# YJxyzxyz/road-vision-system

Hardware: AMD Instinct MI355X
Metric: end-to-end frames/sec @1080p (preproc+YOLOv8n+SORT), 1/2/4/8 MI355X (higher is better)
Workload: dtype bf16

## Files before the change

road-vision-system_amd/csrc/conv.h:

```cpp
#pragma once
#include "common.h"

namespace rv {

typedef uint16_t bf16_t;

struct ConvArgs {
  const bf16_t* in;
  int in_cs, in_co;
  int Hin, Win, Cin;
  const bf16_t* w;
  const float* bias;
  int Cout, k, stride, pad;
  int Ho, Wo, B;
  void* out0;
  int out0_cs, out0_co, out0_up;
  void* out1;
  int out1_cs, out1_co, out1_up;
  int out_f32;
  const bf16_t* res;
  int res_cs, res_co;
  int act;
  int g2_cout0, g2_in_co, g2_Cin;
  const bf16_t* g2_w;
  const float* g2_bias;
  int fused;
  int in8, out0_8, out1_8;
  float s_in, s_res, s_out0, s_out1;
  const float* wscale;
  const float* g2_wscale;
  const bf16_t* in2;
  int in2_cs, in2_co, split, in_up;
  const bf16_t* ch_w;
  const float* ch_b;
};

struct ConvCfg {
  int mr, nr, G, resw, persist;
  int kind = 0;
};

int launch_conv(const ConvArgs& a, hipStream_t s);
int launch_conv_cfg(const ConvArgs& a, const ConvCfg& c, hipStream_t s);
bool conv_cfg_ok(const ConvArgs& a, const ConvCfg& c);
int conv_candidates(const ConvArgs& a, ConvCfg* out, int cap);

struct Conv0Q {
  const int8_t* d;
  const float* s;
  const float* b;
  const int32_t* c;
};
int launch_conv0(const uint8_t* img, int B, int H, int W, const Conv0Q& q, int C0, bf16_t* out,
                 int out_cs, hipStream_t s);
int launch_conv0_fp8(const uint8_t* img, int B, int H, int W, const Conv0Q& q, int C0,
                     uint8_t* out, int out_cs, float s_out, hipStream_t s);

int launch_conv0_k6(const uint8_t* img, int B, int H, int W, const Conv0Q& q, int C0, bf16_t* out,
                    int out_cs, hipStream_t s);

int launch_stem(const uint8_t* img, int B, int H, int W, const Conv0Q& q0, int C0,
                const bf16_t* w1, const float* b1, int C1, bf16_t* out, int out_cs,
                hipStream_t s, const bf16_t* w2 = nullptr, const float* b2 = nullptr,
                bf16_t* out2 = nullptr, int out2_cs = 0, bool k6 = false);

int launch_sppf_pool(bf16_t* buf, int B, int H, int W, int c, hipStream_t s);
int launch_sppf_pool_fp8(uint8_t* buf, int B, int H, int W, int c, hipStream_t s);

struct C2fArgs {
  const bf16_t* cat;
  int cat_cs, cat_co;
  int H, W, B;
  const bf16_t* wa[2];
  const float* ba[2];
  const bf16_t* wb[2];
  const float* bb[2];
  const bf16_t* w2;
  const float* b2;
  bf16_t* out;
  int out_cs, out_co;
  int tap_pairs;
};
bool c2f_fusable(int C, int N, int cat_cs, int cat_co, int out_cs, int out_co);
int launch_c2f_chain(const C2fArgs& a, int C, int N, bool shortcut, hipStream_t s);

struct HeadLevel {
  const float* logits;
  int H, W, cs;
  float stride;
  const bf16_t* feat;
  int feat_cs, cin_b, cin_c;
  const bf16_t* w_box;
  const bf16_t* w_cls;
  const float* b_box;
  const float* b_cls;
  float* logits_out;
};

struct Cand {
  float x1, y1, x2, y2, score;
  int cls, anchor, pad;
};

int decode_segments(const HeadLevel* lv, int nlv);
int launch_detect_decode(const HeadLevel* lv, int nlv, int B, int nc, int reg_max, float conf,
                         float* raw, Cand* cand, int cand_cap, int* seg_n, hipStream_t s,
                         int* form = nullptr, bool cls_only = false);

struct HeadBoxLevel {
  const bf16_t* t;
  int t_cs;
  const bf16_t* w1;
  const float* b1;
};
int launch_head_box(const HeadLevel* lv, const HeadBoxLevel* bx, int nlv, int B, int reg_max,
                    Cand* cand, int cand_cap, const int* seg_n, hipStream_t s);

}
```

road-vision-system_amd/csrc/head_box.hip:

```cpp
#include "conv.h"
#include "conv_common.h"
#include "head.h"

namespace rv {

struct HeadBoxLevels {
  HeadBoxLevel lv[4];
};

constexpr int kBoxC = 64;
constexpr int kURow = kBoxC + 8;
constexpr int kWRowB = 9 * kBoxC * 2 + 16;
constexpr int kWUnits = 9 * kBoxC * 2 / 16;
constexpr int kWPerThread = kBoxC * kWUnits / 256;

template <int REG>
__global__ __launch_bounds__(256) void head_box_kernel(HeadLevels h, HeadBoxLevels hb, int B,
                                                       Cand* __restrict__ cand, int cap,
                                                       const int* __restrict__ seg_n, int nblk) {
  static_assert(4 * REG == kBoxC, "box branch width");
  static_assert(kBoxC * kWUnits % 256 == 0, "weight staging: whole units per thread");
  constexpr int MB = kBoxC / 16, KB = kBoxC / 32;
  extern __shared__ __attribute__((aligned(16))) uint8_t wlds[];
  __shared__ int soff[65];
// ... 28 lines not shown
    b1v[m] = *(const f32x4*)(X.b1 + m * 16 + quad * 4);
    b2v[m] = *(const f32x4*)(L.b_box + m * 16 + quad * 4);
  }
  int n0 = wave == 0 && lane < nsegl ? seg_n[(size_t)b * nblk + blk0 + lane] : 0;
  {
    uint4 wr[kWPerThread];
#pragma unroll
    for (int j = 0; j < kWPerThread; ++j)
      wr[j] = *(const uint4*)(X.w1 + (size_t)(tid + j * 256) * 8);
#pragma unroll
    for (int j = 0; j < kWPerThread; ++j) {
      const int u = tid + j * 256;
      *(uint4*)(wlds + (u / kWUnits) * kWRowB + (u % kWUnits) * 16) = wr[j];
    }
  }
  for (int c0 = 0; c0 < nsegl; c0 += 64) {
    if (wave == 0) {
      const int sgi = c0 + lane;
      int n = c0 == 0 ? n0 : (sgi < nsegl ? seg_n[(size_t)b * nblk + blk0 + sgi] : 0);
      n = min(max(n, 0), 64);
      n = min(n, max(cap - (blk0 + sgi) * 64, 0));
#pragma unroll
      for (int off = 1; off < 64; off <<= 1) {
        const int o = __shfl_up(n, off);
        if (lane >= off) n += o;
      }
      soff[lane + 1] = n;
      if (lane == 0) soff[0] = 0;
    }
    __syncthreads();
    for (int e = tid; e < 64 * 64; e += 256) {
      const int o = soff[e >> 6];
      if ((e & 63) < soff[(e >> 6) + 1] - o) list[o + (e & 63)] = (uint16_t)e;
    }
    __syncthreads();
    const int total = soff[64];
    Cand* const cbase = cand + (size_t)b * cap + (size_t)(blk0 + c0) * 64;
    for (int g0 = z * 4; g0 * 16 < total; g0 += 4 * nz) {
      const int g = g0 + wave;
      const bool active = g * 16 < total;
      int x = 0, y = 0, slot = 0;
      uint4 Bf[KB * 9];
      if (active) {
        const int ci = g * 16 + col;
        slot = list[ci < total ? ci : g * 16];
        int r = cbase[slot].anchor - lstart;
        r = min(max(r, 0), HW - 1);
        y = r / W;
        x = r - y * W;
#pragma unroll
        for (int t = 0; t < 9; ++t) {
          const int yy = y + t / 3 - 1, xx = x + t % 3 - 1;
          const bool in = yy >= 0 && yy < H && xx >= 0 && xx < W;
          const bf16_t* p = tmap + (size_t)(in ? yy * W + xx : 0) * X.t_cs + quad * 8;
#pragma unroll
          for (int k = 0; k < KB; ++k)
            Bf[k * 9 + t] = in ? *(const uint4*)(p + k * 32) : make_uint4(0, 0, 0, 0);
        }
      }
      if (active) {
        f32x4 acc[MB];
#pragma unroll
        for (int m = 0; m < MB; ++m) acc[m] = f32x4{0.f, 0.f, 0.f, 0.f};
#pragma unroll
        for (int k = 0; k < KB; ++k)
#pragma unroll
          for (int t = 0; t < 9; ++t)
#pragma unroll
            for (int m = 0; m < MB; ++m) {
              const uint4 Af = *(const uint4*)(wlds + (m * 16 + col) * kWRowB +
                                               ((t * kBoxC + k * 32 + quad * 8) * 2));
              acc[m] = __builtin_amdgcn_mfma_f32_16x16x32_bf16(
                  __builtin_bit_cast(bf16x8, Af), __builtin_bit_cast(bf16x8, Bf[k * 9 + t]), acc[m],
                  0, 0, 0);
            }
#pragma unroll
        for (int m = 0; m < MB; ++m) {
          float v[4];
#pragma unroll
          for (int i = 0; i < 4; ++i) v[i] = acc[m][i] + b1v[m][i];
          silu4(v);
          *(uint2*)(uw + col * kURow + m * 16 + quad * 4) =
              make_uint2(pack_bf16x2(v[0], v[1]), pack_bf16x2(v[2], v[3]));
        }
      }
      __syncthreads();
      if (active) {
        f32x4 acc[MB];
#pragma unroll
        for (int m = 0; m < MB; ++m) acc[m] = f32x4{0.f, 0.f, 0.f, 0.f};
#pragma unroll
        for (int k = 0; k < KB; ++k) {
          const uint4 Bu = *(const uint4*)(uw + col * kURow + k * 32 + quad * 8);
#pragma unroll
          for (int m = 0; m < MB; ++m)
            acc[m] = __builtin_amdgcn_mfma_f32_16x16x32_bf16(__builtin_bit_cast(bf16x8, Aw[k][m]),
                                                             __builtin_bit_cast(bf16x8, Bu), acc[m],
                                                             0, 0, 0);
        }
#pragma unroll
        for (int m = 0; m < MB; ++m)
          *(f32x4*)(lw + col * (kBoxC + 4) + m * 16 + quad * 4) = acc[m] + b2v[m];
      }
      __syncthreads();
      if (active) {
        const int an = lane >> 2, part = lane & 3;
        const float d = dfl_side<REG>(lw + an * (kBoxC + 4) + part * REG);
        const int base = lane & ~3;
        const float d0 = __shfl(d, base), d1 = __shfl(d, base + 1), d2 = __shfl(d, base + 2),
                    d3 = __shfl(d, base + 3);
        const int xa = __shfl(x, an), ya = __shfl(y, an), sa = __shfl(slot, an);
        if (part == 0 && g * 16 + an < total)
          *(f32x4*)&cbase[sa].x1 = xywh2xyxy(dist2bbox(d0, d1, d2, d3, xa, ya, L.stride));
      }
    }
    __syncthreads();
  }
}

int launch_head_box(const HeadLevel* lv, const HeadBoxLevel* bx, int nlv, int B, int reg_max,
                    Cand* cand, int cand_cap, const int* seg_n, hipStream_t s) {
  HeadLevels h;
  if (!head_levels(lv, nlv, reg_max, h)) return RV_EINVAL;
  HeadBoxLevels hb = {};
  for (int i = 0; i < nlv; ++i) {
    if (!lv[i].w_box || !lv[i].b_box || lv[i].cin_b != kBoxC || !bx[i].t || !bx[i].w1 ||
        !bx[i].b1 || bx[i].t_cs % 8 || (uintptr_t)bx[i].t % 16 || (uintptr_t)bx[i].w1 % 16 ||
        (uintptr_t)bx[i].b1 % 16) {
      set_error("sparse box branch: bad level %d (box width %d)", i, lv[i].cin_b);
      return RV_EINVAL;
    }
    hb.lv[i] = bx[i];
  }
  const int nblk = h.blk[nlv];
  if (!cand || !seg_n || B < 1 || cand_cap < 1 || (uintptr_t)cand % 16) {
    set_error("sparse box branch: candidate buffers incomplete");
    return RV_EINVAL;
  }
  constexpr int smem = kBoxC * kWRowB;
  static const bool raised =
      hipFuncSetAttribute((const void*)head_box_kernel<16>,
                          hipFuncAttributeMaxDynamicSharedMemorySize, smem) == hipSuccess;
  if (!raised) {
    (void)hipGetLastError();
    set_error("sparse box branch: cannot raise the dynamic LDS limit to %d bytes", smem);
    return RV_EINVAL;
  }
  int nz = 4;
  while (nz > 1 && (long)nlv * B * nz > 2L * num_cus()) nz >>= 1;
  head_box_kernel<16><<<dim3(nlv, B, nz), 256, smem, s>>>(h, hb, B, cand, cand_cap, seg_n, nblk);
  return launch_status("head_box");
}

}
```

road-vision-system_amd/csrc/yolo.hip:

```cpp
#include <cmath>
#include <cstring>
#include "yolo_model.h"

namespace rv {

static void plan_heads(Model& M) {
  const Variant& v = M.def.v;
  for (int i = 0; i < 3; ++i) {
    const std::string l = std::to_string(i);
    M.DA[i] = M.newbuf("DA" + l, 3 + i, v.c2d + v.c3p);
    M.DB[i] = M.newbuf("DB" + l, 3 + i, v.c2d + v.c3p, false, true);
    M.HD[i] = M.newbuf("HD" + l, 3 + i, v.hcs, true);
  }
  M.nA = M.map_h[3] * M.map_w[3] + M.map_h[4] * M.map_w[4] + M.map_h[5] * M.map_w[5];
}

static void plan_v5u(Model& M) {
  const Variant& v = M.def.v;
  M.CAT14 = M.CAT11 = -1;
  M.X0 = M.newbuf("X0", 1, v.c1);
  M.X1 = M.newbuf("X1", 2, v.c2);
  M.C2 = M.newbuf("C2", 2, v.c2);
  M.X2 = M.newbuf("X2", 2, v.c2);
  M.X3 = M.newbuf("X3", 3, v.c3);
  M.C4 = M.newbuf("C4", 3, v.c3);
  M.X4 = M.newbuf("X4", 3, v.c3);
  M.X5 = M.newbuf("X5", 4, v.c4);
  M.C6 = M.newbuf("C6", 4, v.c4);
  M.X6 = M.newbuf("X6", 4, v.c4);
  M.X7 = M.newbuf("X7", 5, v.c5);
  M.C8 = M.newbuf("C8", 5, v.c5);
  M.X8 = M.newbuf("X8", 5, v.c5);
  M.SP = M.newbuf("SP", 5, 4 * (v.c5 / 2));
  M.X9 = M.newbuf("X9", 5, v.c5);
  M.CAT20 = M.newbuf("CAT20", 5, 2 * v.c4);
  M.C12 = M.newbuf("C12", 4, v.c4);
  M.X13 = M.newbuf("X13", 4, v.c4);
  M.CAT17 = M.newbuf("CAT17", 4, 2 * v.c3);
  M.C15 = M.newbuf("C15", 3, v.c3);
  M.X15 = M.newbuf("X15", 3, v.c3);
  M.C18 = M.newbuf("C18", 4, v.c4);
  M.X18 = M.newbuf("X18", 4, v.c4);
  M.C21 = M.newbuf("C21", 5, v.c5);
  M.X21 = M.newbuf("X21", 5, v.c5);
  plan_heads(M);
  struct C3Def {
    const char* p;
    int level, c2, n;
  };
  const C3Def cs[] = {{"model.2", 2, v.c2, v.nb},  {"model.4", 3, v.c3, v.nm},
                      {"model.6", 4, v.c4, v.nx},  {"model.8", 5, v.c5, v.nb},
                      {"model.13", 4, v.c4, v.nb}, {"model.17", 3, v.c3, v.nb},
                      {"model.20", 4, v.c4, v.nb}, {"model.23", 5, v.c5, v.nb}};
  for (const C3Def& c : cs)
    for (int i = 0; i < c.n; ++i) {
      M.newbuf(std::string(c.p) + ".t." + std::to_string(i), c.level, c.c2 / 2);
      M.newbuf(std::string(c.p) + ".m." + std::to_string(i), c.level, c.c2 / 2);
    }
}

static void plan(Model& M) {
  const Variant& v = M.def.v;
  for (int i = 0; i < 6; ++i) {
    M.map_h[i] = M.H >> i;
    M.map_w[i] = M.W >> i;
  }
  if (v.family == kFamilyV5u) return plan_v5u(M);
  M.X0 = M.newbuf("X0", 1, v.c1);
  M.X1 = M.newbuf("X1", 2, v.c2);
  M.C2 = M.newbuf("C2", 2, (2 + v.nb) * (v.c2 / 2));
  M.X2 = M.newbuf("X2", 2, v.c2);
  M.X3 = M.newbuf("X3", 3, v.c3);
  M.C4 = M.newbuf("C4", 3, (2 + v.nm) * (v.c3 / 2));
  M.CAT14 = M.newbuf("CAT14", 3, v.h12 + v.c3);
  M.X5 = M.newbuf("X5", 4, v.c4);
  M.C6 = M.newbuf("C6", 4, (2 + v.nm) * (v.c4 / 2));
  M.CAT11 = M.newbuf("CAT11", 4, v.c5 + v.c4);
  M.X7 = M.newbuf("X7", 5, v.c5);
  M.C8 = M.newbuf("C8", 5, (2 + v.nb) * (v.c5 / 2));
  M.X8 = M.newbuf("X8", 5, v.c5);
  M.SP = M.newbuf("SP", 5, 4 * (v.c5 / 2));
  M.CAT20 = M.newbuf("CAT20", 5, v.h18 + v.c5);
  M.C12 = M.newbuf("C12", 4, (2 + v.nb) * (v.h12 / 2));
  M.CAT17 = M.newbuf("CAT17", 4, v.h15 + v.h12);
  M.C15 = M.newbuf("C15", 3, (2 + v.nb) * (v.h15 / 2));
  M.X15 = M.newbuf("X15", 3, v.h15);
  M.C18 = M.newbuf("C18", 4, (2 + v.nb) * (v.h18 / 2));
  M.X18 = M.newbuf("X18", 4, v.h18);
  M.C21 = M.newbuf("C21", 5, (2 + v.nb) * (v.h21 / 2));
  M.X21 = M.newbuf("X21", 5, v.h21);
  plan_heads(M);
  struct C2fDef {
    const char* p;
    int level, c2, n;
  };
  const C2fDef cs[] = {{"model.2", 2, v.c2, v.nb},  {"model.4", 3, v.c3, v.nm},
                       {"model.6", 4, v.c4, v.nm},  {"model.8", 5, v.c5, v.nb},
                       {"model.12", 4, v.h12, v.nb}, {"model.15", 3, v.h15, v.nb},
                       {"model.18", 4, v.h18, v.nb}, {"model.21", 5, v.h21, v.nb}};
  for (const C2fDef& c : cs)
    for (int i = 0; i < c.n; ++i)
      M.newbuf(std::string(c.p) + ".m." + std::to_string(i), c.level, c.c2 / 2);
}

static const View NO_VIEW{-1, 0, 0};

constexpr float kSparseAutoConf = 0.1f;
constexpr int kSparseAutoBatch = 8;

struct ConvIO {
  View in;
  int li;
  View o0;
  int up0 = 0;
  View o1 = NO_VIEW;
  int up1 = 0;
  View res = NO_VIEW;
  const VIn* vin = nullptr;
};

struct Exec {
  Model* M;
  uint8_t* ws;
  int B;
  hipStream_t s;
  std::vector<size_t> off;
  int status = 0;
  bool f8, fusing;
  bool fuse_c2f, fuse_c2f32;
  int cat14, cat11, cat20, cat17;

  Exec(Model* m, void* ws_, int B_, void* stream, std::vector<size_t> off_, bool raw)
      : M(m), ws((uint8_t*)ws_), B(B_), s(as_stream(stream)), off(std::move(off_)) {
    const Variant& v = M->def.v;
    f8 = M->def.dtype == RV_YOLO_DTYPE_FP8;
    fusing = !f8 && !(raw && M->raw_unfused);
    fuse_c2f = fusing && M->fuse_c2f;
    fuse_c2f32 = fuse_c2f && M->fuse_c2f == 2;
    cat14 = v.h12 + v.c3, cat11 = v.c5 + v.c4, cat20 = v.h18 + v.c5, cat17 = v.h15 + v.h12;
    if (v.family == kFamilyV5u) cat14 = cat17 = 2 * v.c3, cat11 = cat20 = 2 * v.c4;
  }

  void* ptr(int buf) const { return ws + off[buf]; }
  const bf16_t* wptr(const ConvSpec& c) const { return (const bf16_t*)(M->dev + c.w_off); }
  const float* bptr(const ConvSpec& c) const { return (const float*)(M->dev + c.b_off); }
  const float* wsptr(const ConvSpec& c) const {
    return c.f8 ? (const float*)(M->dev + c.ws_off) : nullptr;
  }
  float scale(int buf) const { return buf >= 0 ? M->act_scale[buf] : 1.0f; }

  const ConvSpec* spec(const std::string& name) {
    const int idx = M->def.find(name);
    if (idx < 0 && !status) {
      set_error("plan: unknown conv %s", name.c_str());
      status = RV_EINVAL;
    }
    return idx < 0 ? nullptr : &M->def.convs[idx];
  }
  int index(const ConvSpec& c) const { return (int)(&c - M->def.convs.data()); }

  static int out_dim(const ConvSpec& c, int n) { return (n + 2 * (c.k / 2) - c.k) / c.s + 1; }

  ConvArgs args(const ConvSpec& c, const ConvIO& io) const {
    const View in = io.vin ? io.vin->a : io.in, o0 = io.o0, o1 = io.o1, res = io.res;
    ConvArgs a = {};
    a.in = (const bf16_t*)ptr(in.buf);
    a.in_cs = in.cs;
    a.in_co = in.co;
    a.Hin = M->map_h[io.li];
    a.Win = M->map_w[io.li];
    a.Cin = c.pcin;
    a.w = wptr(c);
    a.bias = bptr(c);
    a.Cout = c.pcout;
    a.k = c.k;
    a.stride = c.s;
    a.pad = c.k / 2;
    a.Ho = out_dim(c, a.Hin);
    a.Wo = out_dim(c, a.Win);
    a.B = B;
    a.out0 = ptr(o0.buf);
    a.out0_cs = o0.cs;
    a.out0_co = o0.co;
    a.out0_up = io.up0;
    if (o1.buf >= 0) {
      a.out1 = ptr(o1.buf);
      a.out1_cs = o1.cs;
      a.out1_co = o1.co;
      a.out1_up = io.up1;
    }
    a.out_f32 = M->bufs[o0.buf].f32 ? 1 : 0;
    if (res.buf >= 0) {
      a.res = (const bf16_t*)ptr(res.buf);
      a.res_cs = res.cs;
      a.res_co = res.co;
    }
    a.act = c.act;
    if (c.f8) {
      a.in8 = 1;
      a.s_in = scale(in.buf);
      a.wscale = wsptr(c);
      a.out0_8 = M->bufs[o0.buf].esize == 1;
      a.s_out0 = scale(o0.buf);
      if (o1.buf >= 0) {
        a.out1_8 = M->bufs[o1.buf].esize == 1;
        a.s_out1 = scale(o1.buf);
      }
      if (res.buf >= 0) a.s_res = scale(res.buf);
    }
    if (io.vin) {
      a.in_up = io.vin->up;
      a.in2 = (const bf16_t*)ptr(io.vin->b.buf);
      a.in2_cs = io.vin->b.cs;
      a.in2_co = io.vin->b.co;
      a.split = io.vin->split;
    }
    return a;
  }

  void trace(const ConvSpec& c, const ConvIO& io) {
    const VIn* vi = io.vin;
    const int Hin = M->map_h[io.li], Win = M->map_w[io.li];
    M->trace.push_back(TraceRec{index(c), vi ? vi->a : io.in, Hin, Win, out_dim(c, Hin),
                                out_dim(c, Win), io.o0, io.up0, io.o1, io.up1, io.res,
                                vi ? vi->up : 0, vi ? vi->b : NO_VIEW, vi ? vi->split : 0});
  }

  static double launch_bytes(const ConvArgs& a) {
    const double px_in = (double)a.B * a.Hin * a.Win, px_out = (double)a.B * a.Ho * a.Wo;
    if (a.split > 0 || a.in_up) {
      const double cin1 = a.split > 0 ? a.split : a.Cin;
      const double src = (a.in_up ? px_in / 4 : px_in) * cin1 + px_in * (a.Cin - cin1);
      const double outs = (a.out0 ? (a.out0_up ? 4 : 1) : 0) + (a.out1 ? (a.out1_up ? 4 : 1) : 0);
      return 2.0 * src + 2.0 * px_out * a.Cout * outs + 2.0 * a.Cout * a.Cin;
    }
    const bool g2 = a.g2_cout0 > 0;
    const int cout1 = g2 ? a.g2_cout0 : a.Cout, cout2 = g2 ? a.Cout - a.g2_cout0 : 0;
    double in_ch = a.Cin;
    if (g2 && (a.g2_in_co != a.in_co || a.g2_Cin != a.Cin)) in_ch += a.g2_Cin;
    const double eb = a.in8 ? 1.0 : 2.0;
    auto ob = [&](int o8) { return a.out_f32 ? 4.0 : (o8 ? 1.0 : 2.0); };
    const double outs = (a.out0 ? (a.out0_up ? 4 : 1) * ob(a.out0_8) : 0) +
                        (a.out1 ? (a.out1_up ? 4 : 1) * ob(a.out1_8) : 0);
    const double w = eb * a.k * a.k * ((double)cout1 * a.Cin + (double)cout2 * (g2 ? a.g2_Cin : 0)) +
                     (a.ch_w ? 2.0 * a.Cout * a.Cout : 0.0);
    return px_in * in_ch * eb + px_out * a.Cout * outs + (a.res ? px_out * a.Cout * eb : 0.0) + w;
  }

  double flops_of(const ConvSpec& c, int li) const {
    return 2.0 * B * out_dim(c, M->map_h[li]) * out_dim(c, M->map_w[li]) * (double)c.cout * c.cin *
           c.k * c.k;
  }

  void launch(const ConvArgs& a, const ConvSpec& c, double flops, double bytes) {
    const int li_ = M->li_base + (int)M->launches.size();
    M->launches.push_back(a);
    status = M->prof.timed(li_, s, index(c), flops, bytes, [&] {
      if (a.fused > 0) {
        const Model::FusedC2f& f = M->fused[a.fused - 1];
        return launch_c2f_chain(f.a, f.C, f.N, f.shortcut, s);
      }
// ... 158 lines not shown
  Model* M = E.M;
  const Variant& v = M->def.v;
  const View x0{M->X0, v.c1, 0}, x1{M->X1, v.c2, 0}, x2{M->X2, v.c2, 0};
  const ConvSpec& c0 = M->def.convs[0];
  const uint8_t* qb = M->dev + M->def.q_off;
  const float* qs = (const float*)(qb + 9 * (size_t)c0.cout * 64);
  const Conv0Q q0{(const int8_t*)qb, qs, qs + c0.cout, (const int32_t*)(qs + 2 * c0.cout)};
  const double px0 = (double)E.B * M->map_h[1] * M->map_w[1];
  const double px1 = (double)E.B * M->map_h[2] * M->map_w[2];
  const double f0 = 2.0 * px0 * c0.cout * 108, by_in = (double)E.B * M->H * M->W * 3 + M->def.q_bytes;
  const int slot = M->prof.per_fwd - 1;
  const int i1 = M->def.find("model.1");
  if (E.fusing && M->stem6_fused && c0.cout == 16 && v.c2 == 32 && i1 >= 0) {
    const ConvSpec& c1 = M->def.convs[i1];
    E.trace(c1, {x0, 1, x1});
    E.status = M->prof.timed(slot, E.s, 0, f0 + 2.0 * px1 * c1.cout * c1.cin * 9,
                             by_in + px1 * 2.0 * c1.cout + 2.0 * c1.cout * 9 * 32, [&] {
                               return launch_stem(lb, E.B, M->H, M->W, q0, c0.cout, E.wptr(c1),
                                                  E.bptr(c1), c1.cout, (bf16_t*)E.ptr(M->X1), v.c2,
                                                  E.s, nullptr, nullptr, nullptr, 0, true);
                             });
  } else {
    E.status = M->prof.timed(slot, E.s, 0, f0, by_in + px0 * 2.0 * c0.cout, [&] {
      return launch_conv0_k6(lb, E.B, M->H, M->W, q0, c0.cout, (bf16_t*)E.ptr(M->X0), v.c1, E.s);
    });
    E.conv("model.1", {x0, 1, x1});
  }
  E.c3("model.2", {x1, 2, x2}, M->C2, v.c2, v.nb, true);
  return E.status;
}

static int seg_backbone_v5u(Exec& E) {
  Model* M = E.M;
  const Variant& v = M->def.v;
  const int sc = v.c5 / 2;
  const View x2{M->X2, v.c2, 0}, x3{M->X3, v.c3, 0}, p3{M->X4, v.c3, 0}, x5{M->X5, v.c4, 0},
      p4{M->X6, v.c4, 0}, x7{M->X7, v.c5, 0}, x8{M->X8, v.c5, 0}, sp{M->SP, 4 * sc, 0},
      x9{M->X9, v.c5, 0}, x13{M->X13, v.c4, 0};
  const View t10{M->CAT20, E.cat20, v.c4}, t14{M->CAT17, E.cat17, v.c3};
  const VIn vin13{t10, 1, p4, v.c4}, vin17{t14, 1, p3, v.c3};
  E.conv("model.3", {x2, 2, x3});
  E.c3("model.4", {x3, 3, p3}, M->C4, v.c3, v.nm, true);
  E.conv("model.5", {p3, 3, x5});
  E.c3("model.6", {x5, 4, p4}, M->C6, v.c4, v.nx, true);
  E.conv("model.7", {p4, 4, x7});
  E.c3("model.8", {x7, 5, x8}, M->C8, v.c5, v.nb, true);
  E.conv("model.9.cv1", {x8, 5, sp});
  if (!E.status)
    E.status = launch_sppf_pool((bf16_t*)E.ptr(M->SP), E.B, M->map_h[5], M->map_w[5], sc, E.s);
  E.conv("model.9.cv2", {sp, 5, x9});
  E.conv("model.10", {x9, 5, t10});
  E.c3("model.13", {t10, 4, x13, 0, NO_VIEW, 0, NO_VIEW, &vin13}, M->C12, v.c4, v.nb, false);
  E.conv("model.14", {x13, 4, t14});
  E.c3("model.17", {t14, 3, View{M->X15, v.h15, 0}, 0, NO_VIEW, 0, NO_VIEW, &vin17}, M->C15, v.c3,
       v.nb, false);
  return E.status;
}

static int seg_stem(Exec& E, const uint8_t* lb) {
  Model* M = E.M;
  const Variant& v = M->def.v;
  const int B = E.B;
  const View x0{M->X0, v.c1, 0}, x1{M->X1, v.c2, 0}, x2{M->X2, v.c2, 0};
  const ConvSpec& c0 = M->def.convs[0];
  const uint8_t* qb = M->dev + M->def.q_off;
  const float* qs = (const float*)(qb + 3 * (size_t)c0.cout * 64);
  const Conv0Q q0{(const int8_t*)qb, qs, qs + c0.cout, (const int32_t*)(qs + 2 * c0.cout)};
  const int i1 = M->def.find("model.1");
  const bool fuse_stem = E.fusing && c0.cout == 16 && v.c2 == 32 && i1 >= 0;
  const int i2cv1 = M->def.find("model.2.cv1");
  const int c2cs = E.c2f_will_fuse(v.c2 / 2, v.nb, E.fuse_c2f, 0, NO_VIEW, x2)
                       ? v.c2
                       : (2 + v.nb) * (v.c2 / 2);
  const bool stem_cv1 = fuse_stem && i2cv1 >= 0 && M->def.convs[i2cv1].cin == 32 &&
                        M->def.convs[i2cv1].cout == 32 && M->def.convs[i2cv1].k == 1;
  if (fuse_stem) {
    const ConvSpec& c1 = M->def.convs[i1];
    E.trace(c1, {x0, 1, x1});
    const ConvSpec* cv = stem_cv1 ? &M->def.convs[i2cv1] : nullptr;
    if (cv) E.trace(*cv, {x1, 2, View{M->C2, c2cs, 0}});
    const bool x1_out = !cv || M->stem_x1;
    const double px0 = (double)B * M->map_h[1] * M->map_w[1];
    const double px1 = (double)B * M->map_h[2] * M->map_w[2];
    const double flops = 2.0 * px0 * c0.cout * 27 + 2.0 * px1 * c1.cout * c1.cin * 9 +
                         (cv ? 2.0 * px1 * cv->cout * cv->cin : 0.0);
    const double bytes = (double)B * M->H * M->W * 3 + px1 * 2.0 * (x1_out ? c1.cout : 0) +
                         (cv ? px1 * 2.0 * cv->cout : 0.0) + M->def.q_bytes +
                         2.0 * c1.cout * 9 * 32 + (cv ? 2.0 * cv->cout * 32 : 0.0);
    E.status = M->prof.timed(M->prof.per_fwd - 1, E.s, 0, flops, bytes, [&] {
      return launch_stem(lb, B, M->H, M->W, q0, c0.cout, E.wptr(c1), E.bptr(c1), c1.cout,
                         x1_out ? (bf16_t*)E.ptr(M->X1) : nullptr, v.c2, E.s,
                         cv ? E.wptr(*cv) : nullptr, cv ? E.bptr(*cv) : nullptr,
                         cv ? (bf16_t*)E.ptr(M->C2) : nullptr, c2cs);
    });
  } else {
    E.status = E.f8 ? launch_conv0_fp8(lb, B, M->H, M->W, q0, c0.cout, (uint8_t*)E.ptr(M->X0),
                                       v.c1, E.scale(M->X0), E.s)
                    : launch_conv0(lb, B, M->H, M->W, q0, c0.cout, (bf16_t*)E.ptr(M->X0), v.c1,
                                   E.s);
    E.conv("model.1", {x0, 1, x1});
  }
  E.c2f("model.2", {x1, 2, x2}, M->C2, v.c2, v.nb, true, E.fuse_c2f, stem_cv1);
  return E.status;
}

static int seg_backbone(Exec& E) {
  Model* M = E.M;
  const Variant& v = M->def.v;
  const int cat14 = E.cat14, cat11 = E.cat11, sc = v.c5 / 2;
  const View x2{M->X2, v.c2, 0}, x3{M->X3, v.c3, 0}, x5{M->X5, v.c4, 0}, x7{M->X7, v.c5, 0},
      x8{M->X8, v.c5, 0}, sp{M->SP, 4 * sc, 0};
  const View p3{M->CAT14, cat14, v.h12}, p4{M->CAT11, cat11, v.c5}, p5{M->CAT20, E.cat20, v.h18},
      n4{M->CAT17, E.cat17, v.h15}, c11{M->CAT11, cat11, 0}, c14{M->CAT14, cat14, 0};
  const bool vcat = !E.f8;
  const VIn vin12{p5, 1, p4, v.c5}, vin15{n4, 1, p3, v.h12};
  const int c4 = v.c3 / 2;
  const bool f4 = c4 == 16 ? E.fuse_c2f : E.fuse_c2f32;
  const int c4cs = E.c2f_will_fuse(c4, v.nm, f4, 0, NO_VIEW, p3) ? 2 * c4 : (2 + v.nm) * c4;
  const bool chained = M->fuse_cv1 && E.fusing &&
                       E.conv_chain("model.3", x2, 2, x3, "model.4.cv1", View{M->C4, c4cs, 0});
  if (!chained) E.conv("model.3", {x2, 2, x3});
  E.c2f("model.4", {x3, 3, p3}, M->C4, v.c3, v.nm, true, f4, chained);
  E.conv("model.5", {p3, 3, x5});
  E.c2f("model.6", {x5, 4, p4}, M->C6, v.c4, v.nm, true);
  E.conv("model.7", {p4, 4, x7});
  E.c2f("model.8", {x7, 5, x8}, M->C8, v.c5, v.nb, true);
  E.conv("model.9.cv1", {x8, 5, sp});
  if (!E.status)
    E.status =
        E.f8 ? launch_sppf_pool_fp8((uint8_t*)E.ptr(M->SP), E.B, M->map_h[5], M->map_w[5], sc, E.s)
             : launch_sppf_pool((bf16_t*)E.ptr(M->SP), E.B, M->map_h[5], M->map_w[5], sc, E.s);
  E.conv("model.9.cv2", {sp, 5, p5, 0, vcat ? NO_VIEW : c11, vcat ? 0 : 1});
  E.c2f("model.12", {c11, 4, n4, 0, vcat ? NO_VIEW : c14, vcat ? 0 : 1, NO_VIEW, vcat ? &vin12 : nullptr},
        M->C12, v.h12, v.nb, false);
  E.c2f("model.15", {c14, 3, View{M->X15, v.h15, 0}, 0, NO_VIEW, 0, NO_VIEW, vcat ? &vin15 : nullptr},
        M->C15, v.h15, v.nb, false, v.h15 / 2 == 16 ? E.fuse_c2f : E.fuse_c2f32);
  return E.status;
}

static int seg_heads(Exec& E, float* raw_out, float conf, void* cand, int cand_cap, int* cand_n) {
  Model* M = E.M;
  const Variant& v = M->def.v;
  const int B = E.B;
  const View c17{M->CAT17, E.cat17, 0}, c20{M->CAT20, E.cat20, 0};
  const View P[3] = {View{M->X15, v.h15, 0}, View{M->X18, v.h18, 0}, View{M->X21, v.h21, 0}};
  const int dcs = v.c2d + v.c3p, hcs = v.hcs;
  const bool fuse_head = v.c2d % 8 == 0 && v.c3p % 8 == 0;
  const bool fork =
      M->head_streams && B >= 8 && M->side[0] && M->side[1] && !M->prof.active();
  const hipStream_t main_s = E.s;
  const bool fixed_head = fuse_head && !E.f8 && !raw_out && cand && v.c2d == 64 &&
                          (v.nc == 80 || v.nc <= 64) && v.c3p == (v.nc == 80 ? 80 : 64);
  const bool sparse =
      fixed_head && (M->head_sparse == 1 ||
                     (M->head_sparse == 2 && conf >= kSparseAutoConf && B >= kSparseAutoBatch));
  HeadLevel hl[3] = {};
  HeadBoxLevel hbx[3] = {};
  auto head_level = [&](int i) {
    const std::string a = M->def.head + "cv2." + std::to_string(i),
                      c = M->def.head + "cv3." + std::to_string(i);
    const View da{M->DA[i], dcs, 0}, fb{M->DB[i], dcs, 0}, fc{M->DB[i], dcs, v.c2d},
        lg{M->HD[i], hcs, 0};
    E.conv_pair(a + ".0", P[i], c + ".0", P[i], 3 + i, da);
    if (sparse) {
      const ConvSpec* p1 = E.spec(a + ".1");
      if (!p1) return E.status;
      E.conv_in_sparse(a + ".1", {da, 3 + i, fb});
      E.conv(c + ".1", {View{M->DA[i], dcs, v.c2d}, 3 + i, fc});
      hbx[i] = HeadBoxLevel{(const bf16_t*)E.ptr(M->DA[i]), dcs, E.wptr(*p1), E.bptr(*p1)};
    } else {
      E.conv_pair(a + ".1", da, c + ".1", View{M->DA[i], dcs, v.c2d}, 3 + i, fb);
    }
    HeadLevel& L = hl[i];
    L.logits = (const float*)E.ptr(M->HD[i]);
    L.H = M->map_h[3 + i];
    L.W = M->map_w[3 + i];
    L.cs = hcs;
    L.stride = (float)(8 << i);
    if (!fuse_head) {
      E.conv_pair(a + ".2", fb, c + ".2", fc, 3 + i, lg);
      return E.status;
    }
    const ConvSpec *pa = E.spec(a + ".2"), *pc = E.spec(c + ".2");
    if (!pa || !pc) return E.status;
    const ConvSpec &sa = *pa, &sc = *pc;
    E.trace(sa, {fb, 3 + i, lg});
    E.trace(sc, {fc, 3 + i, View{M->HD[i], hcs, 4 * v.reg}});
    L.feat = (const bf16_t*)E.ptr(M->DB[i]);
    L.feat_cs = dcs;
    L.cin_b = sa.pcin;
    L.cin_c = sc.pcin;
    L.w_box = E.wptr(sa);
    L.w_cls = E.wptr(sc);
    L.b_box = E.bptr(sa);
    L.b_cls = E.bptr(sc);
    L.logits_out = raw_out ? (float*)E.ptr(M->HD[i]) : nullptr;
    return E.status;
  };
  auto forked_head = [&](int i) {
    if (!fork) return head_level(i);
    int e = hip_check(hipEventRecord(M->ev_fork[i], main_s), "head fork hipEventRecord");
    if (!e) e = hip_check(hipStreamWaitEvent(M->side[i], M->ev_fork[i], 0), "head fork wait");
    if (e) return E.status = e;
    E.s = M->side[i];
    const int r = head_level(i);
    e = hip_check(hipEventRecord(M->ev_join[i], M->side[i]), "head join hipEventRecord");
    E.s = main_s;
    if (!r && e) E.status = e;
    return r ? r : e;
  };
  const bool v5 = v.family == kFamilyV5u;
  if (E.status || forked_head(0)) return E.status;
  E.conv(v5 ? "model.18" : "model.16", {P[0], 3, c17});
  if (v5)
    E.c3("model.20", {c17, 4, P[1]}, M->C18, v.h18, v.nb, false);
  else
    E.c2f("model.18", {c17, 4, P[1]}, M->C18, v.h18, v.nb, false);
  if (E.status || forked_head(1)) return E.status;
  E.conv(v5 ? "model.21" : "model.19", {P[1], 4, c20});
  if (v5)
    E.c3("model.23", {c20, 5, P[2]}, M->C21, v.h21, v.nb, false);
  else
    E.c2f("model.21", {c20, 5, P[2]}, M->C21, v.h21, v.nb, false);
  if (E.status || head_level(2)) return E.status;
  if (fork)
    for (int i = 0; i < 2 && !E.status; ++i)
      E.status = hip_check(hipStreamWaitEvent(main_s, M->ev_join[i], 0), "head join wait");
  if (E.status) return E.status;
  if (M->prof.active()) M->prof.n_fwd++;
  const int st = launch_detect_decode(hl, 3, B, v.nc, v.reg, conf, raw_out, (Cand*)cand, cand_cap,
                                      cand_n, E.s, &M->head_form, sparse);
  if (st || !sparse) return st;
  return launch_head_box(hl, hbx, 3, B, v.reg, (Cand*)cand, cand_cap, cand_n, E.s);
}

static int check_resume(const Model& M, int part, int B, const void* ws) {
  if (part != 2 && part != 4) return RV_OK;
  const Resume& r = part == 4 ? M.after_stem : M.after_neck;
  RV_CHECK_ARG(r.n >= 0, "forward part %d before any %s of this handle", part,
               part == 4 ? "part 3" : "part 0 / part 1 forward");
  RV_CHECK_ARG(B == r.B && ws == r.ws,
               "forward part %d (B=%d, ws %p) does not continue the last part %d of this handle "
               "(B=%d, ws %p)", part, B, ws, part == 4 ? 3 : 1, r.B, r.ws);
  return RV_OK;
}

}

using namespace rv;

extern "C" int rv_yolo_create(int variant, const void* dev_packed, int max_B, int in_h, int in_w,
                              void** handle) {
  return rv_yolo_create2(variant, RV_YOLO_DTYPE_BF16, dev_packed, max_B, in_h, in_w, handle);
}

extern "C" int rv_yolo_create2(int variant, int dtype, const void* dev_packed, int max_B, int in_h,
                               int in_w, void** handle) {
  return rv_yolo_create3(variant, dtype, 80, dev_packed, max_B, in_h, in_w, handle);
}

extern "C" int rv_yolo_create3(int variant, int dtype, int nc, const void* dev_packed, int max_B,
                               int in_h, int in_w, void** handle) {
  RV_CHECK_ARG(handle && dev_packed, "null pointer");
  if (const int st = check_plan_args(variant, dtype, nc)) return st;
  RV_CHECK_ARG(max_B > 0 && in_h > 0 && in_w > 0 && in_h % 32 == 0 && in_w % 32 == 0,
               "input %dx%d must be positive multiples of 32", in_h, in_w);
  Model* M = new Model();
  if (!build_def(variant, M->def, dtype, nc)) {
    delete M;
    set_error("unknown variant %d / dtype %d", variant, dtype);
    return RV_EINVAL;
  }
  M->dev = (const uint8_t*)dev_packed;
  for (int i = 0; i < 2; ++i) {
    if (hipStreamCreateWithFlags(&M->side[i], hipStreamNonBlocking) != hipSuccess ||
        hipEventCreateWithFlags(&M->ev_fork[i], hipEventDisableTiming) != hipSuccess ||
        hipEventCreateWithFlags(&M->ev_join[i], hipEventDisableTiming) != hipSuccess) {
      (void)hipGetLastError();
      M->side[0] = M->side[1] = nullptr;
    }
  }
  M->max_B = max_B;
  M->H = in_h;
  M->W = in_w;
  plan(*M);
  M->act_scale.assign(M->bufs.size(), 1.0f);
  M->scales_set = dtype == RV_YOLO_DTYPE_BF16;
  *handle = M;
  return RV_OK;
}

extern "C" int rv_yolo_set_act_scales(void* h, const float* scales, int n) {
  RV_CHECK_ARG(h && scales, "null pointer");
  Model* M = (Model*)h;
  RV_CHECK_ARG(n == (int)M->bufs.size(), "got %d scales, the plan has %d buffers", n,
               (int)M->bufs.size());
  for (int i = 0; i < n; ++i) {
    if (M->bufs[i].esize != 1) continue;
    int e;
    const float f = std::frexp(scales[i], &e);
    RV_CHECK_ARG(scales[i] > 0.f && std::isfinite(scales[i]) && f == 0.5f,
                 "buffer %d: scale %g is not a positive power of two", i, (double)scales[i]);
  }
  for (int i = 0; i < n; ++i) M->act_scale[i] = M->bufs[i].esize == 1 ? scales[i] : 1.0f;
  M->scales_set = true;
  return RV_OK;
}

extern "C" int rv_yolo_buffer_name(void* h, int buf, char* name, int cap) {
  RV_CHECK_ARG(h && name && cap > 0, "bad args");
  Model* M = (Model*)h;
  RV_CHECK_ARG(buf >= 0 && buf < (int)M->bufs.size(), "bad buffer %d", buf);
  strncpy(name, M->bufs[buf].name.c_str(), cap - 1);
  name[cap - 1] = 0;
  return RV_OK;
}

extern "C" int rv_yolo_buffer_esize(void* h, int buf) {
  RV_CHECK_ARG(h, "null handle");
  Model* M = (Model*)h;
  RV_CHECK_ARG(buf >= 0 && buf < (int)M->bufs.size(), "bad buffer %d", buf);
  return M->bufs[buf].esize;
}

extern "C" int rv_yolo_destroy(void* h) {
  delete (Model*)h;
  return RV_OK;
}

extern "C" int rv_yolo_set_option(void* h, int opt, int value) {
  RV_CHECK_ARG(h, "null handle");
  Model* M = (Model*)h;
  switch (opt) {
    case RV_YOLO_OPT_RAW_UNFUSED:
      M->raw_unfused = value != 0;
      return RV_OK;
    case RV_YOLO_OPT_FUSE_C2F:
      M->fuse_c2f = value < 0 ? 0 : (value > 2 ? 2 : value);
      return RV_OK;
    case RV_YOLO_OPT_STEM_X1:
      M->stem_x1 = value != 0;
      return RV_OK;
    case RV_YOLO_OPT_HEAD_STREAMS:
      M->head_streams = value != 0;
      return RV_OK;
    case RV_YOLO_OPT_FUSE_CV1:
      M->fuse_cv1 = value != 0;
      return RV_OK;
    case RV_YOLO_OPT_C2F_TAP_PAIRS:
      M->c2f_tap_pairs = value != 0;
      return RV_OK;
    case RV_YOLO_OPT_STEM6_FUSED:
      M->stem6_fused = value != 0;
      return RV_OK;
    case RV_YOLO_OPT_HEAD_SPARSE:
      RV_CHECK_ARG(value >= 0 && value <= 2, "head sparse option %d not in {0, 1, 2}", value);
      M->head_sparse = value;
      return RV_OK;
    default:
      set_error("unknown yolo option %d", opt);
      return RV_EINVAL;
  }
}

extern "C" size_t rv_yolo_ws_bytes(void* h, int B) {
  if (!h || B <= 0) return 0;
  return ((Model*)h)->ws_bytes(B);
}

extern "C" int rv_yolo_num_anchors(void* h) { return h ? ((Model*)h)->nA : 0; }

extern "C" int rv_yolo_num_classes(void* h) { return h ? ((Model*)h)->def.v.nc : 0; }

extern "C" int rv_yolo_head_form(void* h) { return h ? ((Model*)h)->head_form : RV_EINVAL; }

extern "C" int rv_yolo_cand_segments(void* h) {
  if (!h) return 0;
  const Model* M = (const Model*)h;
  HeadLevel hl[3];
  for (int i = 0; i < 3; ++i) {
    hl[i].H = M->map_h[3 + i];
    hl[i].W = M->map_w[3 + i];
  }
  return decode_segments(hl, 3);
}

extern "C" int rv_yolo_forward(void* h, const uint8_t* lb, int B, void* ws, size_t ws_bytes,
                               float* raw_out, float conf, void* cand, int cand_cap, int* cand_n,
                               void* stream) {
  return rv_yolo_forward_part(h, lb, B, ws, ws_bytes, raw_out, conf, cand, cand_cap, cand_n, stream,
                              0);
}

extern "C" int rv_yolo_forward_part(void* h, const uint8_t* lb, int B, void* ws, size_t ws_bytes,
                                    float* raw_out, float conf, void* cand, int cand_cap,
                                    int* cand_n, void* stream, int part) {
  RV_CHECK_ARG(h && ws && (lb || part == 2 || part == 4), "null pointer");
  RV_CHECK_ARG(part >= 0 && part <= 4, "part %d not in {0, 1, 2, 3, 4}", part);
  Model* M = (Model*)h;
  if (const int st = check_resume(*M, part, B, ws)) return st;
  RV_CHECK_ARG((part != 1 && part != 3 && part != 4) || !raw_out,
               "raw_out needs the whole forward (part 0)");
  RV_CHECK_ARG(B > 0 && B <= M->max_B, "B=%d outside (0, %d]", B, M->max_B);
  std::vector<size_t> off = M->offsets(B);
  RV_CHECK_ARG(ws_bytes >= off.back(), "workspace %zu < %zu bytes", ws_bytes, off.back());
  RV_CHECK_ARG(!cand || (cand_n && cand_cap > 0), "candidate buffers incomplete");
  RV_CHECK_ARG(M->scales_set, "fp8 plan: activation scales not set (rv_yolo_set_act_scales)");
  Exec E(M, ws, B, stream, std::move(off), raw_out != nullptr);
  M->trace.clear();
  M->launches.clear();
  M->fused.clear();
  M->li_base = part == 2 ? M->after_neck.n : (part == 4 ? M->after_stem.n : 0);
  static const int SEGS[5] = {7, 3, 4, 1, 2};
  const int segs = SEGS[part];
  auto here = [&] { return Resume{M->li_base + (int)M->launches.size(), B, ws}; };
  const bool v5 = M->def.v.family == kFamilyV5u;
  if ((segs & 1) && (v5 ? seg_stem_v5u(E, lb) : seg_stem(E, lb))) return E.status;
  if (part == 3) {
    M->after_stem = here();
    M->after_neck = Resume{};
  }
  if (segs & 2) {
    if (v5 ? seg_backbone_v5u(E) : seg_backbone(E)) return E.status;
    M->after_neck = here();
  }
  return (segs & 4) ? seg_heads(E, raw_out, conf, cand, cand_cap, cand_n) : RV_OK;
}

extern "C" int rv_yolo_num_buffers(void* h) { return h ? (int)((Model*)h)->bufs.size() : 0; }

extern "C" int rv_yolo_buffer_info(void* h, int B, int buf, int* info, size_t* off_bytes) {
  RV_CHECK_ARG(h && info && off_bytes && B > 0, "bad args");
  Model* M = (Model*)h;
  RV_CHECK_ARG(buf >= 0 && buf < (int)M->bufs.size(), "bad buffer %d", buf);
  *off_bytes = M->offsets(B)[buf];
  const Buf& b = M->bufs[buf];
  info[0] = b.h;
  info[1] = b.w;
  info[2] = b.c;
  info[3] = b.f32 ? 1 : 0;
  return RV_OK;
}

extern "C" int rv_yolo_trace(void* h, int* recs, int max_recs) {
  if (!h) return RV_EINVAL;
  Model* M = (Model*)h;
  const int n = (int)M->trace.size();
  static_assert(sizeof(TraceRec) == 24 * sizeof(int), "rv_yolo_trace: 24 ints per record");
  if (recs)
    for (int i = 0; i < n && i < max_recs; ++i) memcpy(recs + 24 * i, &M->trace[i], 24 * sizeof(int));
  return n;
}
```

Before: 45850.

## Compute box-branch first conv only at candidate neighbourhoods in sparse head

Adds a sparse path for the first 3x3 conv of the box branch (cv2.i.0). Instead of running it densely over the whole feature map, a new kernel marks the 3x3 neighbourhoods of decoded candidate anchors in an LDS bitmap, compacts them into a position list, and runs MFMA only at those positions. The class-branch conv still runs densely, and a new option value plus auto thresholds (high confidence, large batch) enable the path. It removes dense box-branch work at the cost of an extra launch, atomics and large dynamic LDS, and it only helps when candidates are few.

```diff
diff --git a/road-vision-system_amd/csrc/conv.h b/road-vision-system_amd/csrc/conv.h
--- a/road-vision-system_amd/csrc/conv.h
+++ b/road-vision-system_amd/csrc/conv.h
@@ -116,4 +116,16 @@
 int launch_head_box(const HeadLevel* lv, const HeadBoxLevel* bx, int nlv, int B, int reg_max,
                     Cand* cand, int cand_cap, const int* seg_n, hipStream_t s);
 
+struct HeadPosLevel {
+  const bf16_t* in;
+  int in_cs, cin;
+  const bf16_t* w0;
+  const float* b0;
+  bf16_t* t;
+  int t_cs;
+};
+size_t head_pos_lds(int H, int W, int cin);
+int launch_head_pos(const HeadLevel* lv, const HeadPosLevel* px, int nlv, int B, int reg_max,
+                    const Cand* cand, int cand_cap, const int* seg_n, hipStream_t s);
+
 }
diff --git a/road-vision-system_amd/csrc/head_box.hip b/road-vision-system_amd/csrc/head_box.hip
--- a/road-vision-system_amd/csrc/head_box.hip
+++ b/road-vision-system_amd/csrc/head_box.hip
@@ -204,4 +204,224 @@
   return launch_status("head_box");
 }
 
-}
+struct HeadPosItem {
+  HeadPosLevel p;
+  int H, W, lstart, blk0, nsegl;
+};
+struct HeadPosArgs {
+  HeadPosItem it[3];
+};
+
+constexpr int kPosMaxLds = 160 * 1024;
+constexpr int kPosThreads = 512;
+__host__ __device__ constexpr int pos_row_bytes(int cin) { return 9 * cin * 2 + 16; }
+
+template <int KB>
+__device__ __forceinline__ void head_pos_level(const HeadPosItem& I, uint8_t* lds, int b, int z,
+                                               int nz, const Cand* __restrict__ cand, int cap,
+                                               const int* __restrict__ seg_n, int nblk) {
+  constexpr int CIN = KB * 32, ROWB = pos_row_bytes(CIN), UNITS = 9 * CIN * 2 / 16;
+  constexpr int MB = kBoxC / 16, NT = kPosThreads, NWV = NT / 64, WPER = kBoxC * UNITS / NT;
+  constexpr int U = 8;
+  static_assert(kBoxC * UNITS == NT * WPER, "weight staging: whole units per thread");
+  const int tid = threadIdx.x, wave = tid >> 6, lane = tid & 63, col = lane & 15, quad = lane >> 4;
+  const int H = I.H, W = I.W, HW = H * W, nW = (HW + 31) >> 5, nsegl = I.nsegl;
+  uint32_t* const bm = (uint32_t*)(lds + kBoxC * ROWB);
+  int* const woff = (int*)(bm + nW);
+  uint16_t* const plist = (uint16_t*)(woff + nW + 1);
+  for (int w = tid; w < nW; w += NT) bm[w] = 0;
+  __syncthreads();
+  const int* const sn = seg_n + (size_t)b * nblk + I.blk0;
+  const Cand* const cbase = cand + (size_t)b * cap + (size_t)I.blk0 * 64;
+  const int nslot = nsegl * 64;
+  auto counts = [&](int e0, int (&n)[U]) {
+#pragma unroll
+    for (int u = 0; u < U; ++u) {
+      const int e = e0 + u * NT;
+      n[u] = e < nslot ? sn[e >> 6] : 0;
+    }
+  };
+  auto anchors = [&](int e0, const int (&n)[U], int (&an)[U], bool (&ok)[U]) {
+#pragma unroll
+    for (int u = 0; u < U; ++u) {
+      const int e = e0 + u * NT, sg = e >> 6;
+      const int c = min(min(max(n[u], 0), 64), max(cap - (I.blk0 + sg) * 64, 0));
+      ok[u] = e < nslot && (e & 63) < c;
+      an[u] = ok[u] ? cbase[e].anchor : 0;
+    }
+  };
+  auto mark = [&](const int (&an)[U], const bool (&ok)[U]) {
+#pragma unroll
+    for (int u = 0; u < U; ++u) {
+      if (!ok[u]) continue;
+      const int r = min(max(an[u] - I.lstart, 0), HW - 1);
+      const int y = r / W, x = r - y * W;
+      for (int yy = max(y - 1, 0); yy <= min(y + 1, H - 1); ++yy)
+        for (int xx = max(x - 1, 0); xx <= min(x + 1, W - 1); ++xx) {
+          const int p = yy * W + xx;
+          atomicOr(&bm[p >> 5], 1u << (p & 31));
+        }
+    }
+  };
+  int n[U], an[U];
+  bool ok[U];
+  counts(tid, n);
+  f32x4 b0v[MB];
+#pragma unroll
+  for (int m = 0; m < MB; ++m) b0v[m] = *(const f32x4*)(I.p.b0 + m * 16 + quad * 4);
+  {
+    uint4 wr[WPER];
+#pragma unroll
+    for (int j = 0; j < WPER; ++j)
+      wr[j] = *(const uint4*)(I.p.w0 + (size_t)(tid + j * NT) * 8);
+    anchors(tid, n, an, ok);
+#pragma unroll
+    for (int j = 0; j < WPER; ++j) {
+      const int u = tid + j * NT;
+      *(uint4*)(lds + (u / UNITS) * ROWB + (u % UNITS) * 16) = wr[j];
+    }
+  }
+  mark(an, ok);
+  for (int e0 = tid + U * NT; e0 < nslot; e0 += U * NT) {
+    counts(e0, n);
+    anchors(e0, n, an, ok);
+    mark(an, ok);
+  }
+  __syncthreads();
+  if (wave == 0) {
+    int run = 0;
+    for (int w0 = 0; w0 < nW; w0 += 64) {
+      const int c = w0 + lane < nW ? __popc(bm[w0 + lane]) : 0;
+      int inc = c;
+#pragma unroll
+      for (int off = 1; off < 64; off <<= 1) {
+        const int o = __shfl_up(inc, off);
+        if (lane >= off) inc += o;
+      }
+      if (w0 + lane < nW) woff[w0 + lane] = run + inc - c;
+      run += __shfl(inc, 63);
+    }
+    if (lane == 0) woff[nW] = run;
+  }
+  __syncthreads();
+  for (int w = tid; w < nW; w += NT) {
+    uint32_t bits = bm[w];
+    int o = woff[w];
+    while (bits) {
+      const int p = w * 32 + __ffs(bits) - 1;
+      if (p < HW) plist[o] = (uint16_t)p;
+      ++o;
+      bits &= bits - 1;
+    }
+  }
+  __syncthreads();
+  const int total = min(woff[nW], HW);
+  const bf16_t* const imap = I.p.in + (size_t)b * HW * I.p.in_cs;
+  bf16_t* const tmap = I.p.t + (size_t)b * HW * I.p.t_cs;
+  for (int g = z * NWV + wave; g * 16 < total; g += NWV * nz) {
+    const int ci = g * 16 + col;
+    const int pos = min((int)plist[ci < total ? ci : g * 16], HW - 1);
+    const int y = pos / W, x = pos - y * W;
+    uint4 Bf[KB * 9];
+#pragma unroll
+    for (int k = 0; k < KB; ++k)
+#pragma unroll
+      for (int t = 0; t < 9; ++t) {
+        const int yy = y + t / 3 - 1, xx = x + t % 3 - 1;
+        const bool in = yy >= 0 && yy < H && xx >= 0 && xx < W;
+        const bf16_t* p = imap + (size_t)(in ? yy * W + xx : 0) * I.p.in_cs + k * 32 + quad * 8;
+        Bf[k * 9 + t] = in ? *(const uint4*)p : make_uint4(0, 0, 0, 0);
+      }
+    f32x4 acc[MB];
+#pragma unroll
+    for (int m = 0; m < MB; ++m) acc[m] = f32x4{0.f, 0.f, 0.f, 0.f};
+#pragma unroll
+    for (int k = 0; k < KB; ++k) {
+#pragma unroll
+      for (int t = 0; t < 9; ++t)
+#pragma unroll
+        for (int m = 0; m < MB; ++m) {
+          const uint4 Af =
+              *(const uint4*)(lds + (m * 16 + col) * ROWB + ((t * CIN + k * 32 + quad * 8) * 2));
+          acc[m] = __builtin_amdgcn_mfma_f32_16x16x32_bf16(__builtin_bit_cast(bf16x8, Af),
+                                                           __builtin_bit_cast(bf16x8, Bf[k * 9 + t]),
+                                                           acc[m], 0, 0, 0);
+        }
+      __builtin_amdgcn_sched_barrier(0);
+    }
+    if (ci < total) {
+#pragma unroll
+      for (int m = 0; m < MB; ++m) {
+        float v[4];
+#pragma unroll
+        for (int i = 0; i < 4; ++i) v[i] = acc[m][i] + b0v[m][i];
+        silu4(v);
+        *(uint2*)(tmap + (size_t)pos * I.p.t_cs + m * 16 + quad * 4) =
+            make_uint2(pack_bf16x2(v[0], v[1]), pack_bf16x2(v[2], v[3]));
+      }
+    }
+  }
+}
+
+__global__ __launch_bounds__(kPosThreads) void head_pos_kernel(HeadPosArgs a,
+                                                               const Cand* __restrict__ cand, int cap,
+                                                               const int* __restrict__ seg_n,
+                                                               int nblk) {
+  extern __shared__ __attribute__((aligned(16))) uint8_t plds[];
+  HeadPosItem I = a.it[0];
+#pragma unroll
+  for (int i = 1; i < 3; ++i)
+    if (i == (int)blockIdx.x) I = a.it[i];
+  if (I.p.cin == 64)
+    head_pos_level<2>(I, plds, blockIdx.y, blockIdx.z, gridDim.z, cand, cap, seg_n, nblk);
+  else
+    head_pos_level<4>(I, plds, blockIdx.y, blockIdx.z, gridDim.z, cand, cap, seg_n, nblk);
+}
+
+size_t head_pos_lds(int H, int W, int cin) {
+  if ((cin != 64 && cin != 128) || H < 1 || W < 1 || (long)H * W > 65536) return 0;
+  const int HW = H * W, nW = (HW + 31) >> 5;
+  const size_t bytes = (size_t)kBoxC * pos_row_bytes(cin) + 4 * (size_t)(nW + nW + 1) + 2 * (size_t)HW;
+  return bytes <= (size_t)kPosMaxLds ? bytes : 0;
+}
+
+int launch_head_pos(const HeadLevel* lv, const HeadPosLevel* px, int nlv, int B, int reg_max,
+                    const Cand* cand, int cand_cap, const int* seg_n, hipStream_t s) {
+  HeadLevels h;
+  if (!head_levels(lv, nlv, reg_max, h)) return RV_EINVAL;
+  if (!cand || !seg_n || B < 1 || cand_cap < 1) {
+    set_error("sparse cv2.i.0: candidate buffers incomplete");
+    return RV_EINVAL;
+  }
+  HeadPosArgs a = {};
+  int n = 0;
+  size_t smem = 0;
+  for (int i = 0; i < nlv; ++i) {
+    const HeadPosLevel& p = px[i];
+    if (!p.in) continue;
+    const size_t need = head_pos_lds(lv[i].H, lv[i].W, p.cin);
+    if (n >= 3 || !need || !p.w0 || !p.b0 || !p.t || p.in_cs % 8 || p.in_cs < p.cin || p.t_cs % 4 ||
+        p.t_cs < kBoxC || (uintptr_t)p.in % 16 || (uintptr_t)p.w0 % 16 || (uintptr_t)p.b0 % 16 ||
+        (uintptr_t)p.t % 8) {
+      set_error("sparse cv2.i.0: bad level %d (%dx%d, cin %d)", i, lv[i].H, lv[i].W, p.cin);
+      return RV_EINVAL;
+    }
+    a.it[n++] = HeadPosItem{p, lv[i].H, lv[i].W, h.start[i], h.blk[i], h.blk[i + 1] - h.blk[i]};
+    smem = std::max(smem, need);
+  }
+  if (!n) return RV_OK;
+  static const bool raised =
+      hipFuncSetAttribute((const void*)head_pos_kernel, hipFuncAttributeMaxDynamicSharedMemorySize,
+                          kPosMaxLds) == hipSuccess;
+  if (!raised) {
+    (void)hipGetLastError();
+    set_error("sparse cv2.i.0: cannot raise the dynamic LDS limit to %d bytes", kPosMaxLds);
+    return RV_EINVAL;
+  }
+  int nz = 4;
+  while (nz > 1 && (long)n * B * nz > (long)num_cus()) nz >>= 1;
+  head_pos_kernel<<<dim3(n, B, nz), kPosThreads, smem, s>>>(a, cand, cand_cap, seg_n, h.blk[nlv]);
+  return launch_status("head_pos");
+}
+
+}
diff --git a/road-vision-system_amd/csrc/yolo.hip b/road-vision-system_amd/csrc/yolo.hip
--- a/road-vision-system_amd/csrc/yolo.hip
+++ b/road-vision-system_amd/csrc/yolo.hip
@@ -107,6 +107,8 @@
 
 constexpr float kSparseAutoConf = 0.1f;
 constexpr int kSparseAutoBatch = 8;
+constexpr float kSparse0AutoConf = 0.3f;
+constexpr int kSparse0AutoBatch = 128;
 
 struct ConvIO {
   View in;
@@ -571,16 +573,30 @@
   const bool fixed_head = fuse_head && !E.f8 && !raw_out && cand && v.c2d == 64 &&
                           (v.nc == 80 || v.nc <= 64) && v.c3p == (v.nc == 80 ? 80 : 64);
   const bool sparse =
-      fixed_head && (M->head_sparse == 1 ||
+      fixed_head && (M->head_sparse == 1 || M->head_sparse == 3 ||
                      (M->head_sparse == 2 && conf >= kSparseAutoConf && B >= kSparseAutoBatch));
+  const bool sparse0 =
+      sparse && (M->head_sparse == 3 || (M->head_sparse == 2 && conf >= kSparse0AutoConf &&
+                                         B >= kSparse0AutoBatch));
   HeadLevel hl[3] = {};
   HeadBoxLevel hbx[3] = {};
+  HeadPosLevel hpx[3] = {};
   auto head_level = [&](int i) {
     const std::string a = M->def.head + "cv2." + std::to_string(i),
                       c = M->def.head + "cv3." + std::to_string(i);
     const View da{M->DA[i], dcs, 0}, fb{M->DB[i], dcs, 0}, fc{M->DB[i], dcs, v.c2d},
         lg{M->HD[i], hcs, 0};
-    E.conv_pair(a + ".0", P[i], c + ".0", P[i], 3 + i, da);
+    const ConvSpec* p0 = sparse0 ? E.spec(a + ".0") : nullptr;
+    if (sparse0 && !p0) return E.status;
+    if (p0 && p0->k == 3 && p0->s == 1 && p0->act && p0->pcout == v.c2d && p0->pcin == P[i].cs &&
+        head_pos_lds(M->map_h[3 + i], M->map_w[3 + i], p0->pcin)) {
+      E.conv_in_sparse(a + ".0", {P[i], 3 + i, da});
+      E.conv(c + ".0", {P[i], 3 + i, View{da.buf, da.cs, da.co + v.c2d}});
+      hpx[i] = HeadPosLevel{(const bf16_t*)E.ptr(P[i].buf) + P[i].co, P[i].cs, p0->pcin, E.wptr(*p0),
+                            E.bptr(*p0), (bf16_t*)E.ptr(M->DA[i]), dcs};
+    } else {
+      E.conv_pair(a + ".0", P[i], c + ".0", P[i], 3 + i, da);
+    }
     if (sparse) {
       const ConvSpec* p1 = E.spec(a + ".1");
       if (!p1) return E.status;
@@ -650,6 +666,11 @@
   const int st = launch_detect_decode(hl, 3, B, v.nc, v.reg, conf, raw_out, (Cand*)cand, cand_cap,
                                       cand_n, E.s, &M->head_form, sparse);
   if (st || !sparse) return st;
+  if (hpx[0].in || hpx[1].in || hpx[2].in) {
+    if (const int sp = launch_head_pos(hl, hpx, 3, B, v.reg, (const Cand*)cand, cand_cap, cand_n, E.s))
+      return sp;
+    M->head_form = 4;
+  }
   return launch_head_box(hl, hbx, 3, B, v.reg, (Cand*)cand, cand_cap, cand_n, E.s);
 }
 
@@ -773,7 +794,7 @@
       M->stem6_fused = value != 0;
       return RV_OK;
     case RV_YOLO_OPT_HEAD_SPARSE:
-      RV_CHECK_ARG(value >= 0 && value <= 2, "head sparse option %d not in {0, 1, 2}", value);
+      RV_CHECK_ARG(value >= 0 && value <= 3, "head sparse option %d not in {0, 1, 2, 3}", value);
       M->head_sparse = value;
       return RV_OK;
     default:
```

Result: slower. 45190 (-1.4%).
